# stevesuyao/KinectDepthMapEnhancement

Measured on AMD Instinct MI355X. Metric: Mpixels/sec joint-bilateral filtered (640x480 & 1080p); % HBM roofline, higher is better.
Workload: dtype f32; 1 GPU; JointBilateralFilter::Process (K0 pre-smooth 5/30/30 + K1) on 64 x 640x480 synthetic RGB-D frames (64 per GPU), window 11 (radius 5), sigma_s 3 px, sigma_r 7.65/255, sigma_d 20 mm; frames_per_gpu=64, width=640, height=480, window=11, kernel_variant=auto (w11-pk2-16x16-false-v4)

## Files before the change

### kinectdepthmapenhancement_amd/csrc/jbf_kernels.hip

```cpp
#include "kde_internal.h"
#include "kde_device_math.h"
#include "kde_device_packed.h"

namespace kde {
namespace {

constexpr int kTileX = 32;
constexpr int kTileY = 8;
constexpr int kThreads = kTileX * kTileY;

__device__ __forceinline__ int color_dist2(uint32_t a, uint32_t b)
{
    int d0 = (int)(a & 0xffu) - (int)(b & 0xffu);
    int d1 = (int)((a >> 8) & 0xffu) - (int)((b >> 8) & 0xffu);
    int d2 = (int)((a >> 16) & 0xffu) - (int)((b >> 16) & 0xffu);
    return d0 * d0 + d1 * d1 + d2 * d2;
}

__device__ __forceinline__ int reflect101(int p, int len)
{
    if (len == 1) return 0;
    while (p < 0 || p >= len) {
        if (p < 0) p = -p;
        else p = 2 * len - 2 - p;
    }
    return p;
}

struct JbfDev {
    const float* depth;
    const uint8_t* guide;
    float* out;
    const float* s_eff;
    int width, height, window;
    float color_den, depth_den;
    int color_on, depth_on;
    int cd_skip;
    float d2_skip;
    KDE_STAGE(float* stage_avg;)
};

__global__ __launch_bounds__(kThreads) void jbf_generic_kernel(JbfDev a)
{
    extern __shared__ __attribute__((aligned(16))) unsigned char smem[];
    const int R = a.window / 2;
    const int LW = kTileX + 2 * R, LH = kTileY + 2 * R;
    float* sd = reinterpret_cast<float*>(smem);
    uint32_t* sc = reinterpret_cast<uint32_t*>(sd + LW * LH);
    float* ss = reinterpret_cast<float*>(sc + LW * LH);

    const size_t frame = (size_t)blockIdx.z * a.width * a.height;
    const float* __restrict__ depth = a.depth + frame;
    const uint8_t* __restrict__ guide = a.guide + frame * 3;
    const int x0 = blockIdx.x * kTileX, y0 = blockIdx.y * kTileY;
    const int tid = threadIdx.x;

    for (int i = tid; i < LW * LH; i += kThreads) {
        const int ly = i / LW, lx = i - ly * LW;
        const int gx = x0 + lx - R, gy = y0 + ly - R;
        float d = 0.0f;
        uint32_t c = 0;
        if (gx >= 0 && gx < a.width && gy >= 0 && gy < a.height) {
            const size_t q = (size_t)gy * a.width + gx;
            d = depth[q];
            if (!(d > 50.0f)) d = 0.0f;
            c = load_bgrx(guide, q);
        }
        sd[i] = d;
        sc[i] = c;
    }
    for (int i = tid; i < a.window * a.window; i += kThreads) ss[i] = a.s_eff[i];
    __syncthreads();

    const int tx = tid & (kTileX - 1), ty = tid / kTileX;
    const int x = x0 + tx, y = y0 + ty;
    if (x >= a.width || y >= a.height) return;

    const uint32_t cc = sc[(ty + R) * LW + tx + R];
    float w_average = 0.0f, weight = 0.0f;
    for (int i = 0; i < a.window; i++) {
        for (int j = 0; j < a.window; j++) {
            const int li = (ty + i) * LW + tx + j;
            const float dq = sd[li];
            if (dq > 50.0f) {
                const int cd = color_dist2(cc, sc[li]);
                float filter = ss[i * a.window + j];
                if (a.color_on && cd < a.cd_skip) filter *= exp_denormal(-(float)cd / a.color_den);
                w_average += dq * filter;
                weight += filter;
            }
        }
    }
    float result = 0.0f;
    if (weight > 0.0f) {
        w_average /= weight;
        float numerator = 0.0f, denominator = 0.0f;
        for (int i = 0; i < a.window; i++) {
            for (int j = 0; j < a.window; j++) {
                const int li = (ty + i) * LW + tx + j;
                const float dq = sd[li];
                if (dq > 50.0f) {
                    const int cd = color_dist2(cc, sc[li]);
                    float filter = ss[i * a.window + j];
                    if (a.color_on && cd < a.cd_skip) filter *= exp_denormal(-(float)cd / a.color_den);
                    const float dd = dq - w_average;
                    const float d2 = dd * dd;
                    if (a.depth_on && !(d2 >= a.d2_skip)) filter *= exp_denormal(-d2 / a.depth_den);
                    numerator += dq * filter;
                    denominator += filter;
                }
            }
        }
        result = (denominator == 0.0f) ? 0.0f : numerator / denominator;
    }
    a.out[frame + (size_t)y * a.width + x] = result;
    KDE_STAGE(if (a.stage_avg) a.stage_avg[frame + (size_t)y * a.width + x] = weight > 0.0f ? w_average : __builtin_nanf("");)
}

struct PreDev {
    const uint8_t* src;
    uint8_t* dst;
    const float* lut;
    int width, height, n;
    int tiles_x, tiles_y;
    int band_walk;
    FastDiv24 div_tpf, div_tx;
};

constexpr int kPreBX = 16, kPreBY = 16;

__device__ __forceinline__ uint32_t cvt_pk_u8(float v, uint32_t byte, uint32_t old)
{
    uint32_t r;
    asm("v_cvt_pk_u8_f32 %0, %1, %2, %3" : "=v"(r) : "v"(v), "v"(byte), "v"(old));
    return r;
}
constexpr int kPreTH = kPreBY;

constexpr int kPreRpWaves = 7;
template <int R, int PX>
__global__ __launch_bounds__(kPreBX* kPreBY, (R <= 2 ? kPreRpWaves : 0)) void presmooth_kernel(PreDev a)
{
    constexpr int kPrePX = PX, kPreTW = kPreBX * PX;
    constexpr int NT = kPreBX * kPreBY;
    constexpr int LW = kPreTW + 2 * R, LH = kPreTH + 2 * R;
    constexpr int LUT_N = (R * R + 1) * 766;
    constexpr int SEG = kPrePX + 2 * R;
    __shared__ float lut[LUT_N];
    constexpr int LP = (LW + 3) / 4 * 4;
    __shared__ __attribute__((aligned(16))) uint32_t sc[LH * LP + 4];

    const int tid = threadIdx.x;
    for (int i = tid; i < LUT_N; i += NT) lut[i] = a.lut[i];
    const float w_centre = __uint_as_float(__builtin_amdgcn_readfirstlane(__float_as_uint(a.lut[0])));

    const int tiles_per_frame = a.tiles_x * a.tiles_y;
    const int total = tiles_per_frame * a.n;
    const int tx = tid % kPreBX, ty = tid / kPreBX;

    constexpr int RPP = NT / LW;
    constexpr int NSLOT = (LH + RPP - 1) / RPP;
    const int sy0 = tid / LW, sx = tid - sy0 * LW;
    const bool stager = sy0 < RPP;
    const uint32_t lds0 = (uint32_t)(sy0 * LP + sx);
    const uint32_t rel0 = ((uint32_t)sy0 * (uint32_t)a.width + (uint32_t)sx) * 3u;
    const uint32_t out_rel = ((uint32_t)ty * (uint32_t)a.width + (uint32_t)(tx * kPrePX)) * 3u;
    const size_t last_pix = (size_t)a.n * a.width * a.height - 1;
    auto tile_of = [&](int L) { return a.band_walk ? (int)xcd_band_id((unsigned)L, (unsigned)total) : L; };
    constexpr int kRun = 4;
    const unsigned w_xcd = blockIdx.x % 8u, w_slot = blockIdx.x / 8u;
    const unsigned w_per = (unsigned)total / 8u, w_rem = (unsigned)total % 8u;
    const unsigned w_start = w_xcd * w_per + (w_xcd < w_rem ? w_xcd : w_rem), w_len = w_per + (w_xcd < w_rem ? 1u : 0u);
    const unsigned w_wgs = (gridDim.x + 7u - w_xcd) / 8u;
    const unsigned w_full = a.band_walk == 2 ? w_len / ((unsigned)kRun * w_wgs) : 0u;
    auto tile_index = [&](int it) -> int {
        if (a.band_walk != 2) {
            const long long L = (long long)blockIdx.x + (long long)it * gridDim.x;
            return L < total ? tile_of((int)L) : -1;
        }
        unsigned pos;
        if ((unsigned)it < w_full * kRun) pos = (unsigned)kRun * (w_slot + ((unsigned)it / kRun) * w_wgs) + (unsigned)it % kRun;
        else pos = w_full * kRun * w_wgs + w_slot + ((unsigned)it - w_full * kRun) * w_wgs;
        return pos < w_len ? (int)(w_start + pos) : -1;
    };
    struct TileAt { int frame_i, tyi, txi; };
    auto tile_at = [&](int tile_id) {
        const uint32_t t = (uint32_t)tile_id;
        const uint32_t f = fastdiv24(t, a.div_tpf);
        const uint32_t tile = t - f * (uint32_t)tiles_per_frame;
        const uint32_t ty_ = fastdiv24(tile, a.div_tx);
        return TileAt{(int)f, (int)ty_, (int)(tile - ty_ * (uint32_t)a.tiles_x)};
    };
    auto fetch = [&](const TileAt& at, uint32_t* pre) {
        const int frame_i = at.frame_i, tyi = at.tyi, txi = at.txi;
        const size_t frame = (size_t)frame_i * a.width * a.height;
        const bool ends_batch = frame_i == a.n - 1 && txi * kPreTW + kPreTW + R == a.width && tyi * kPreTH + kPreTH + R == a.height;
        const bool inner = txi * kPreTW - R >= 0 && txi * kPreTW + kPreTW + R <= a.width && tyi * kPreTH - R >= 0 &&
                           tyi * kPreTH + kPreTH + R <= a.height && !ends_batch;
        if (inner) {
            const uint8_t* base = a.src + (frame + (size_t)(tyi * kPreTH - R) * a.width + (size_t)(txi * kPreTW - R)) * 3;
#pragma unroll
            for (int k = 0; k < NSLOT; k++) {
                if (stager && sy0 + k * RPP < LH)
                    __builtin_memcpy(&pre[k], base + (size_t)(k * RPP) * a.width * 3 + rel0, 4);
            }
            return;
        }
#pragma unroll
        for (int k = 0; k < NSLOT; k++) {
            if (stager && sy0 + k * RPP < LH) {
                const int gx = reflect101(txi * kPreTW + sx - R, a.width);
                const int gy = reflect101(tyi * kPreTH + sy0 + k * RPP - R, a.height);
                const size_t pix = frame + (size_t)gy * a.width + gx;
                if (pix < last_pix) __builtin_memcpy(&pre[k], a.src + pix * 3, 4);
                else pre[k] = load_bgrx(a.src, pix);
            }
        }
    };

    uint32_t pre[NSLOT];
    TileAt cur{0, 0, 0};
    int cur_id = tile_index(0);
    if (cur_id >= 0) {
        cur = tile_at(cur_id);
        fetch(cur, pre);
    }
    for (int it = 0; cur_id >= 0; it++) {
        const int frame_i = cur.frame_i;
        const int x0 = cur.txi * kPreTW, y0 = cur.tyi * kPreTH;
        const size_t frame = (size_t)frame_i * a.width * a.height;

        __syncthreads();
#pragma unroll
        for (int k = 0; k < NSLOT; k++)
            if (stager && sy0 + k * RPP < LH) sc[lds0 + k * RPP * LP] = pre[k] & 0x00ffffffu;
        __syncthreads();
        cur_id = tile_index(it + 1);
        if (cur_id >= 0) {
            cur = tile_at(cur_id);
            fetch(cur, pre);
        }

        const bool full = x0 + kPreTW <= a.width && y0 + kPreTH <= a.height;
        const int xb = x0 + tx * kPrePX, y = y0 + ty;
        if (!full && (xb >= a.width || y >= a.height)) continue;

        uint32_t cc[kPrePX];
        f2 sbg[kPrePX];
        float sr[kPrePX], sden[kPrePX];
#pragma unroll
        for (int k = 0; k < kPrePX; k++) {
            cc[k] = sc[(ty + R) * LP + tx * kPrePX + R + k];
            sbg[k] = f2{0.0f, 0.0f};
            sr[k] = sden[k] = 0.0f;
        }
#pragma unroll
        for (int dy = -R; dy <= R; dy++) {
            uint32_t v[(SEG + 3) / 4 * 4];
            f2 fbg[SEG];
            float fr[SEG];
            if (PX == 4) {
#pragma unroll
                for (int q4 = 0; q4 < (SEG + 3) / 4; q4++) {
                    const uint4 w = *reinterpret_cast<const uint4*>(&sc[(ty + R + dy) * LP + tx * kPrePX + 4 * q4]);
                    v[4 * q4] = w.x; v[4 * q4 + 1] = w.y; v[4 * q4 + 2] = w.z; v[4 * q4 + 3] = w.w;
                }
            } else {
#pragma unroll
                for (int q2 = 0; q2 < (SEG + 1) / 2; q2++) {
                    const uint2 w = *reinterpret_cast<const uint2*>(&sc[(ty + R + dy) * LP + tx * kPrePX + 2 * q2]);
                    v[2 * q2] = w.x; v[2 * q2 + 1] = w.y;
                }
            }
#pragma unroll
            for (int q = 0; q < SEG; q++) {
                fbg[q] = f2{(float)(v[q] & 0xffu), (float)((v[q] >> 8) & 0xffu)};
                fr[q] = (float)((v[q] >> 16) & 0xffu);
            }
#pragma unroll
            for (int dx = -R; dx <= R; dx++) {
                const int space2 = dx * dx + dy * dy;
                if (space2 > R * R) continue;
#pragma unroll
                for (int k = 0; k < kPrePX; k++) {
                    const int q = k + R + dx;
                    float w;
                    if (space2 == 0) {
                        w = w_centre;
                    } else {
                        const uint32_t n1 = __builtin_amdgcn_sad_u8(v[q], cc[k], 0u);
                        w = lut[space2 * 766 + n1];
                    }
                    sbg[k] = __builtin_elementwise_fma(f2{w, w}, fbg[q], sbg[k]);
                    sr[k] = __builtin_fmaf(w, fr[q], sr[k]);
                    sden[k] += w;
                }
            }
        }
        uint32_t px[kPrePX];
#pragma unroll
        for (int k = 0; k < kPrePX; k++) {
            const float den = sden[k];
            const float r = __builtin_amdgcn_rcpf(den);
            const f2 qbg = sbg[k] * f2{r, r};
            float q[3] = {qbg.x, qbg.y, sr[k] * r};
            const f2 ebg = f2{__builtin_amdgcn_fractf(q[0]), __builtin_amdgcn_fractf(q[1])} - f2{0.5f, 0.5f};
            const float er = __builtin_amdgcn_fractf(q[2]) - 0.5f;
            const float emin = __builtin_fminf(__builtin_fminf(__builtin_fabsf(ebg.x), __builtin_fabsf(ebg.y)), __builtin_fabsf(er));
            const bool ambiguous = !(emin > 1.0e-4f) || !__builtin_amdgcn_class(den, 0x100);
            if (ambiguous) {
                q[0] = sbg[k].x / den;
                q[1] = sbg[k].y / den;
                q[2] = sr[k] / den;
            }
            px[k] = cvt_pk_u8(q[2], 2u, cvt_pk_u8(q[1], 1u, cvt_pk_u8(q[0], 0u, 0u)));
        }
        uint8_t* o = a.dst + (frame + (size_t)y0 * a.width + x0) * 3 + out_rel;
        if (PX == 4 && (a.width & 3) == 0 && xb + 3 < a.width && (reinterpret_cast<uintptr_t>(a.dst) & 3u) == 0) {
            uint32_t* ow = reinterpret_cast<uint32_t*>(o);
            ow[0] = px[0] | (px[1] << 24);
            ow[1] = (px[1] >> 8) | (px[2] << 16);
            ow[2] = (px[2] >> 16) | (px[3 % PX] << 8);
        } else if (PX == 2 && (full || xb + 1 < a.width)) {
            const uint16_t h0 = (uint16_t)(px[0] & 0xffffu), h1 = (uint16_t)((px[0] >> 16) | ((px[1] & 0xffu) << 8)),
                           h2 = (uint16_t)(px[1] >> 8);
            __builtin_memcpy(o, &h0, 2);
            __builtin_memcpy(o + 2, &h1, 2);
            __builtin_memcpy(o + 4, &h2, 2);
        } else {
#pragma unroll
            for (int k = 0; k < kPrePX; k++)
                if (xb + k < a.width) {
                    o[3 * k] = (uint8_t)(px[k] & 0xff);
                    o[3 * k + 1] = (uint8_t)((px[k] >> 8) & 0xff);
                    o[3 * k + 2] = (uint8_t)((px[k] >> 16) & 0xff);
                }
        }
    }
}

__global__ __launch_bounds__(kPreBX* kPreBY) void presmooth_generic_kernel(PreDev a, int R)
{
    const int x = blockIdx.x * kPreBX + threadIdx.x % kPreBX, y = blockIdx.y * kPreBY + threadIdx.x / kPreBX;
    if (x >= a.width || y >= a.height) return;
    const size_t frame = (size_t)blockIdx.z * a.width * a.height;
    const uint32_t cc = load_bgrx(a.src, frame + (size_t)y * a.width + x);
    float s0 = 0.0f, s1 = 0.0f, s2 = 0.0f, sum2 = 0.0f;
    for (int dy = -R; dy <= R; dy++) {
        const int gy = reflect101(y + dy, a.height);
        for (int dx = -R; dx <= R; dx++) {
            const int space2 = dx * dx + dy * dy;
            if (space2 > R * R) continue;
            const uint32_t v = load_bgrx(a.src, frame + (size_t)gy * a.width + reflect101(x + dx, a.width));
            const uint32_t n1 = __builtin_amdgcn_sad_u8(v, cc, 0u);
            const float w = a.lut[(size_t)space2 * 766 + n1];
            s0 = __builtin_fmaf(w, (float)(v & 0xffu), s0);
            s1 = __builtin_fmaf(w, (float)((v >> 8) & 0xffu), s1);
            s2 = __builtin_fmaf(w, (float)((v >> 16) & 0xffu), s2);
            sum2 += w;
        }
    }
    auto sat = [](float q) -> uint8_t {
        if (!(q > 0.0f)) return 0;
        if (q >= 255.0f) return 255;
        return (uint8_t)rintf(q);
    };
    uint8_t* o = a.dst + (frame + (size_t)y * a.width + x) * 3;
    o[0] = sat(s0 / sum2);
    o[1] = sat(s1 / sum2);
    o[2] = sat(s2 / sum2);
}

struct MrfDev {
    const float* depth;
    const uint8_t* bgr;
    float* out;
    int width, height, window;
    float color_sigma, smooth_sigma;
};

__global__ __launch_bounds__(kThreads) void mrf_kernel(MrfDev a)
{
    extern __shared__ __attribute__((aligned(16))) unsigned char smem[];
    const int R = a.window / 2;
    const int LW = kTileX + 2 * R, LH = kTileY + 2 * R;
    float* sd = reinterpret_cast<float*>(smem);
    uint32_t* sc = reinterpret_cast<uint32_t*>(sd + LW * LH);

    const size_t frame = (size_t)blockIdx.z * a.width * a.height;
    const float* __restrict__ depth = a.depth + frame;
    const uint8_t* __restrict__ bgr = a.bgr + frame * 3;
    const int x0 = blockIdx.x * kTileX, y0 = blockIdx.y * kTileY;
    const int tid = threadIdx.x;

    for (int i = tid; i < LW * LH; i += kThreads) {
        const int ly = i / LW, lx = i - ly * LW;
        const int gx = x0 + lx - R, gy = y0 + ly - R;
        float d = 0.0f;
        uint32_t c = 0;
        if (gx >= 0 && gx < a.width && gy >= 0 && gy < a.height) {
            const size_t q = (size_t)gy * a.width + gx;
            d = depth[q];
            if (!(d > 50.0f)) d = 0.0f;
            c = load_bgrx(bgr, q);
        }
        sd[i] = d;
        sc[i] = c;
    }
    __syncthreads();

    const int tx = tid & (kTileX - 1), ty = tid / kTileX;
    const int x = x0 + tx, y = y0 + ty;
    if (x >= a.width || y >= a.height) return;

    const uint32_t cc = sc[(ty + R) * LW + tx + R];
    float numerator = depth[(size_t)y * a.width + x], denominator = 1.0f;
    for (int i = 0; i < a.window; i++) {
        for (int j = 0; j < a.window; j++) {
            const int li = (ty + i) * LW + tx + j;
            const float dq = sd[li];
            if (dq > 50.0f) {
                const int cd = color_dist2(cc, sc[li]);
                float color_filter = 0.0f;
                if (a.color_sigma != 0.0f) color_filter = exp_denormal(-a.color_sigma * (float)cd);
                float filter = a.smooth_sigma;
                filter *= color_filter;
                numerator += dq * filter;
                denominator += filter;
            }
        }
    }
    a.out[frame + (size_t)y * a.width + x] = (denominator == 0.0f) ? 0.0f : numerator / denominator;
}

}

int jbf_variant_count() { return 1 + jbf_fast_variant_count(); }
const char* jbf_variant_name(int v) { return v == 0 ? "generic-32x8-1px" : jbf_fast_variant_name(v - 1); }

int jbf_active_variant(const JbfLaunch& a)
{
    if (a.variant > 0) return a.variant;
    if (a.variant < 0 && jbf_fast_supported(a)) return 1 + jbf_fast_default_variant(a);
    return 0;
}

int launch_jbf(const JbfLaunch& a, hipStream_t s)
{
    if (a.variant > 0) {
        if (!jbf_fast_supported(a)) return fail(KDE_ERR_INVALID, "jbf: tuned variants need non-zero sigmas and a built window");
        return launch_jbf_fast(a, a.variant - 1, a.table_host, s);
    }
    if (a.variant < 0 && jbf_fast_supported(a))
        return launch_jbf_fast(a, jbf_fast_default_variant(a), a.table_host, s);
    JbfDev d;
    d.depth = a.depth;
    d.guide = a.guide;
    d.out = a.out;
    d.s_eff = a.s_eff;
    d.width = a.width;
    d.height = a.height;
    d.window = a.window;
    d.color_den = a.color_den;
    d.depth_den = a.depth_den;
    d.color_on = a.color_sigma != 0.0f;
    d.depth_on = a.depth_sigma != 0.0f;
    d.cd_skip = a.cd_skip;
    d.d2_skip = a.d2_skip;
    KDE_STAGE(d.stage_avg = g_stage.jbf_avg;)
    const int R = a.window / 2;
    const size_t lds = (size_t)(kTileX + 2 * R) * (kTileY + 2 * R) * 8 + (size_t)a.window * a.window * 4;
    dim3 grid(ceil_div(a.width, kTileX), ceil_div(a.height, kTileY), a.n);
    hipLaunchKernelGGL(jbf_generic_kernel, grid, dim3(kThreads), lds, s, d);
    KDE_HIP_TRY(hipGetLastError());
    return KDE_OK;
}

constexpr int kPrePxPerThread = 2;

long long presmooth_resident_blocks(int radius)
{
    auto resident = [](auto kernel) -> long long {
        int dev = 0, cus = 0, per_cu = 0;
        if (hipGetDevice(&dev) != hipSuccess ||
            hipDeviceGetAttribute(&cus, hipDeviceAttributeMultiprocessorCount, dev) != hipSuccess ||
            hipOccupancyMaxActiveBlocksPerMultiprocessor(&per_cu, kernel, kPreBX * kPreBY, 0) != hipSuccess ||
            cus <= 0 || per_cu <= 0) {
            (void)hipGetLastError();
            return 256;
        }
        return (long long)cus * per_cu;
    };
    switch (radius) {
        case 1: return resident(presmooth_kernel<1, kPrePxPerThread>);
        case 2: return resident(presmooth_kernel<2, kPrePxPerThread>);
        case 3: return resident(presmooth_kernel<3, kPrePxPerThread>);
        case 4: return resident(presmooth_kernel<4, kPrePxPerThread>);
        default: return 0;
    }
}

static int k0_band_walk(int width, int height, int n)
{
    return (long long)width * height * n * 3 <= (32ll << 20) ? 1 : 2;
}

int launch_presmooth(const PresmoothLaunch& a, hipStream_t s)
{
    PreDev d;
    d.src = a.src;
    d.dst = a.dst;
    d.lut = a.lut;
    d.width = a.width;
    d.height = a.height;
    d.n = a.n;
    constexpr int kPX = kPrePxPerThread;
    d.band_walk = k0_band_walk(a.width, a.height, a.n);
    d.tiles_x = ceil_div(a.width, kPreBX * kPX);
    d.tiles_y = ceil_div(a.height, kPreTH);
    if (a.radius < 1) return fail(KDE_ERR_INVALID, "presmooth: radius %d", a.radius);
    if (a.radius > 4) {
        if (a.n > 65535) return fail(KDE_ERR_INVALID, "presmooth: batch too large for one launch");
        hipLaunchKernelGGL(presmooth_generic_kernel, dim3(ceil_div(a.width, kPreBX), ceil_div(a.height, kPreBY), a.n),
                           dim3(kPreBX * kPreBY), 0, s, d, a.radius);
        KDE_HIP_TRY(hipGetLastError());
        return KDE_OK;
    }
    const long long total = (long long)d.tiles_x * d.tiles_y * a.n;
    if (total > 0x7fffffffLL) return fail(KDE_ERR_INVALID, "presmooth: batch too large for one launch");
    d.div_tpf = make_fastdiv24((uint32_t)(d.tiles_x * d.tiles_y), (uint64_t)total);
    d.div_tx = make_fastdiv24((uint32_t)d.tiles_x, (uint64_t)d.tiles_x * d.tiles_y);
    const long long cap = a.grid_cap > 0 ? a.grid_cap : 256;
    const unsigned grid = (unsigned)(total < cap ? total : cap);
    if (d.band_walk == 2 && grid < 8) d.band_walk = 1;
    switch (a.radius) {
        case 1: hipLaunchKernelGGL((presmooth_kernel<1, kPX>), dim3(grid), dim3(kPreBX * kPreBY), 0, s, d); break;
        case 2: hipLaunchKernelGGL((presmooth_kernel<2, kPX>), dim3(grid), dim3(kPreBX * kPreBY), 0, s, d); break;
        case 3: hipLaunchKernelGGL((presmooth_kernel<3, kPX>), dim3(grid), dim3(kPreBX * kPreBY), 0, s, d); break;
        default: hipLaunchKernelGGL((presmooth_kernel<4, kPX>), dim3(grid), dim3(kPreBX * kPreBY), 0, s, d); break;
    }
    KDE_HIP_TRY(hipGetLastError());
    return KDE_OK;
}

struct MrfFastDev {
    const float* depth;
    const uint8_t* bgr;
    float* out;
    int width, height;
    float kc;
    float lsm;
    float unscale;
};

constexpr int kMrfBX = 32, kMrfBY = 8, kMrfPX = 2;

template <int WIN>
__global__ __launch_bounds__(kMrfBX* kMrfBY) void mrf_fast_kernel(MrfFastDev a)
{
    constexpr int R = WIN / 2, NT = kMrfBX * kMrfBY, TW = kMrfBX * kMrfPX, TH = kMrfBY;
    constexpr int LW = TW + 2 * R, LH = TH + 2 * R;
    constexpr uint32_t kMagicM = 0x4B000000u, kOffM = 1u << 18, kInvalidM = 0xFF000000u;
    constexpr float kBiasM = 8388608.0f + 262144.0f;
    __shared__ __attribute__((aligned(8))) float s_d[LH * LW];
    __shared__ __attribute__((aligned(8))) uint32_t s_c[LH * LW];
    __shared__ __attribute__((aligned(8))) uint32_t s_n[LH * LW];

    const size_t frame = (size_t)blockIdx.z * a.width * a.height;
    const float* __restrict__ depth = a.depth + frame;
    const uint8_t* __restrict__ bgr = a.bgr + frame * 3;
    const int x0 = blockIdx.x * TW, y0 = blockIdx.y * TH;
    const int tid = threadIdx.x;
    for (int i = tid; i < LW * LH; i += NT) {
        const int ly = i / LW, lx = i - ly * LW;
        const int gx = x0 + lx - R, gy = y0 + ly - R;
        float d = 0.0f;
        uint32_t c = 0;
        if (gx >= 0 && gx < a.width && gy >= 0 && gy < a.height) {
            const size_t q = (size_t)gy * a.width + gx;
            d = depth[q];
            c = load_bgrx(bgr, q);
        }
        const bool valid = d > 50.0f;
        s_d[i] = valid ? d : 0.0f;
        s_c[i] = c;
        s_n[i] = valid ? (kMagicM + kOffM) - __builtin_amdgcn_udot4(c, c, 0u, false) : kInvalidM;
    }
    __syncthreads();

    const int tx = tid % kMrfBX, ty = tid / kMrfBX;
    const int xb = x0 + tx * kMrfPX, y = y0 + ty;
    if (xb >= a.width || y >= a.height) return;
    static_assert(kMrfPX == 2 && LW % 2 == 0, "pair geometry");
    constexpr int SEGP = 1 + R;
    uint32_t cc[2];
    f2 negC, num = {0.0f, 0.0f}, den = {0.0f, 0.0f};
#pragma unroll
    for (int k = 0; k < 2; k++) {
        cc[k] = s_c[(ty + R) * LW + tx * 2 + R + k];
        negC[k] = -(kBiasM + (float)__builtin_amdgcn_udot4(cc[k], cc[k], 0u, false));
    }
    const f2 kc2 = {a.kc, a.kc}, lsm2 = {a.lsm, a.lsm};
#pragma unroll
    for (int i = 0; i < WIN; i++) {
        f2 dp[SEGP];
        uint2 cp[SEGP], np[SEGP];
#pragma unroll
        for (int m = 0; m < SEGP; m++) {
            const int li = (ty + i) * LW + tx * 2 + 2 * m;
            dp[m] = *reinterpret_cast<const f2*>(&s_d[li]);
            cp[m] = *reinterpret_cast<const uint2*>(&s_c[li]);
            np[m] = *reinterpret_cast<const uint2*>(&s_n[li]);
        }
#pragma unroll
        for (int u = 0; u < WIN; u++) {
            uint32_t c0, c1, n0, n1;
            pair_unit_pick(cp, WIN, u, 0, c0, c1);
            pair_unit_pick(np, WIN, u, 0, n0, n1);
            const f2 dq = pair_unit_pick(dp, WIN, u);
            const uint32_t u0 = (__builtin_amdgcn_udot4(c0, cc[0], 0u, false) << 1) + n0;
            const uint32_t u1 = (__builtin_amdgcn_udot4(c1, cc[1], 0u, false) << 1) + n1;
            const f2 ncd = f2{__uint_as_float(u0), __uint_as_float(u1)} + negC;
            const f2 arg = __builtin_elementwise_fma(ncd, kc2, lsm2);
            const f2 f = {__builtin_amdgcn_exp2f(arg.x), __builtin_amdgcn_exp2f(arg.y)};
            num = __builtin_elementwise_fma(dq, f, num);
            den = den + f;
        }
    }
    float* __restrict__ o = a.out + frame + (size_t)y * a.width + xb;
#pragma unroll
    for (int k = 0; k < kMrfPX; k++)
        if (xb + k < a.width) {
            const float n = __builtin_fmaf(num[k], a.unscale, depth[(size_t)y * a.width + xb + k]);
            const float d = __builtin_fmaf(den[k], a.unscale, 1.0f);
            o[k] = (d == 0.0f) ? 0.0f : n / d;
        }
}

int launch_mrf(const MrfLaunch& a, hipStream_t s)
{
    if (a.window == 5 && a.color_sigma > 0.0f && a.smooth_sigma >= 0.0f && a.color_sigma < 1.0e30f && a.smooth_sigma < 1.0e30f) {
        MrfFastDev f;
        f.depth = a.depth; f.bgr = a.bgr; f.out = a.out; f.width = a.width; f.height = a.height;
        f.kc = (float)((double)a.color_sigma * 1.4426950408889634);
        const double lsm = a.smooth_sigma == 0.0f ? -INFINITY : std::log2((double)a.smooth_sigma);
        const int off = lsm + 32.0 < 120.0 ? 32 : 0;
        f.lsm = (float)(lsm + off);
        f.unscale = (float)std::ldexp(1.0, -off);
        dim3 fgrid(ceil_div(a.width, kMrfBX * kMrfPX), ceil_div(a.height, kMrfBY), a.n);
        hipLaunchKernelGGL(mrf_fast_kernel<5>, fgrid, dim3(kMrfBX * kMrfBY), 0, s, f);
        KDE_HIP_TRY(hipGetLastError());
        return KDE_OK;
    }
    MrfDev d{a.depth, a.bgr, a.out, a.width, a.height, a.window, a.color_sigma, a.smooth_sigma};
    const int R = a.window / 2;
    const size_t lds = (size_t)(kTileX + 2 * R) * (kTileY + 2 * R) * 8;
    dim3 grid(ceil_div(a.width, kTileX), ceil_div(a.height, kTileY), a.n);
    hipLaunchKernelGGL(mrf_kernel, grid, dim3(kThreads), lds, s, d);
    KDE_HIP_TRY(hipGetLastError());
    return KDE_OK;
}

}
```

Baseline: 18150 Mpixels/s.

## Pre-convert presmooth LDS tile to float4, compact LUT, faster border fetch

The presmooth kernel now stores each staged pixel in LDS as a float4 holding the three channels already converted to float plus the packed bits, so the inner loop skips per-row unpacking and int-to-float conversion. The spatial LUT is compacted to only the squared distances that actually occur, shrinking its LDS footprint. Border tiles take a cheaper reflect path using 32-bit offsets, and the exact-division fallback for ambiguous rounding is grouped behind a single branch. The cost is a 4x larger LDS tile, which raises LDS traffic and may lower occupancy.

```diff
diff --git a/kinectdepthmapenhancement_amd/csrc/jbf_kernels.hip b/kinectdepthmapenhancement_amd/csrc/jbf_kernels.hip
--- a/kinectdepthmapenhancement_amd/csrc/jbf_kernels.hip
+++ b/kinectdepthmapenhancement_amd/csrc/jbf_kernels.hip
@@ -25,6 +25,13 @@
         else p = 2 * len - 2 - p;
     }
     return p;
+}
+
+__device__ __forceinline__ int reflect_near(int p, int len)
+{
+    p = p < 0 ? -p : p;
+    p = p >= len ? 2 * len - 2 - p : p;
+    return p < 0 ? 0 : p;
 }
 
 struct JbfDev {
@@ -136,6 +143,24 @@
     return r;
 }
 constexpr int kPreTH = kPreBY;
+typedef float f4 __attribute__((ext_vector_type(4)));
+
+struct PreRowMap {
+    int row[17];
+    int n;
+};
+constexpr PreRowMap make_pre_row_map(int R)
+{
+    PreRowMap m{};
+    for (int s2 = 0; s2 < 17; s2++) m.row[s2] = -1;
+    for (int s2 = 1; s2 <= R * R; s2++) {
+        bool occurs = false;
+        for (int dy = 0; dy <= R; dy++)
+            for (int dx = 0; dx <= R; dx++) occurs = occurs || dx * dx + dy * dy == s2;
+        if (occurs) m.row[s2] = m.n++;
+    }
+    return m;
+}
 
 constexpr int kPreRpWaves = 7;
 template <int R, int PX>
@@ -144,14 +169,17 @@
     constexpr int kPrePX = PX, kPreTW = kPreBX * PX;
     constexpr int NT = kPreBX * kPreBY;
     constexpr int LW = kPreTW + 2 * R, LH = kPreTH + 2 * R;
-    constexpr int LUT_N = (R * R + 1) * 766;
     constexpr int SEG = kPrePX + 2 * R;
-    __shared__ float lut[LUT_N];
-    constexpr int LP = (LW + 3) / 4 * 4;
-    __shared__ __attribute__((aligned(16))) uint32_t sc[LH * LP + 4];
+    constexpr PreRowMap kRows = make_pre_row_map(R);
+    __shared__ float lut[kRows.n * 766];
+    constexpr int LP = LW | 1;
+    __shared__ __attribute__((aligned(16))) f4 sc[LH * LP];
 
     const int tid = threadIdx.x;
-    for (int i = tid; i < LUT_N; i += NT) lut[i] = a.lut[i];
+#pragma unroll
+    for (int s2 = 1; s2 <= R * R; s2++)
+        if (kRows.row[s2] >= 0)
+            for (int i = tid; i < 766; i += NT) lut[kRows.row[s2] * 766 + i] = a.lut[s2 * 766 + i];
     const float w_centre = __uint_as_float(__builtin_amdgcn_readfirstlane(__float_as_uint(a.lut[0])));
 
     const int tiles_per_frame = a.tiles_x * a.tiles_y;
@@ -191,6 +219,7 @@
         const uint32_t ty_ = fastdiv24(tile, a.div_tx);
         return TileAt{(int)f, (int)ty_, (int)(tile - ty_ * (uint32_t)a.tiles_x)};
     };
+    const bool border_fast = a.width > R && a.height > R && (unsigned long long)a.width * (unsigned long long)a.height * 3ull < (1ull << 32);
     auto fetch = [&](const TileAt& at, uint32_t* pre) {
         const int frame_i = at.frame_i, tyi = at.tyi, txi = at.txi;
         const size_t frame = (size_t)frame_i * a.width * a.height;
@@ -206,6 +235,22 @@
             }
             return;
         }
+        if (border_fast) {
+            const uint8_t* fbase = a.src + frame * 3;
+            const bool has_last = frame_i == a.n - 1 && txi * kPreTW + kPreTW + R >= a.width && tyi * kPreTH + kPreTH + R >= a.height;
+            const uint32_t last_off = ((uint32_t)a.width * (uint32_t)a.height - 1u) * 3u;
+            const int gx = reflect_near(txi * kPreTW + sx - R, a.width);
+#pragma unroll
+            for (int k = 0; k < NSLOT; k++) {
+                if (stager && sy0 + k * RPP < LH) {
+                    const int gy = reflect_near(tyi * kPreTH + sy0 + k * RPP - R, a.height);
+                    const uint32_t off = ((uint32_t)gy * (uint32_t)a.width + (uint32_t)gx) * 3u;
+                    if (has_last && off == last_off) pre[k] = load_bgrx(fbase, (size_t)gy * a.width + gx);
+                    else __builtin_memcpy(&pre[k], fbase + off, 4);
+                }
+            }
+            return;
+        }
 #pragma unroll
         for (int k = 0; k < NSLOT; k++) {
             if (stager && sy0 + k * RPP < LH) {
@@ -233,7 +278,10 @@
         __syncthreads();
 #pragma unroll
         for (int k = 0; k < NSLOT; k++)
-            if (stager && sy0 + k * RPP < LH) sc[lds0 + k * RPP * LP] = pre[k] & 0x00ffffffu;
+            if (stager && sy0 + k * RPP < LH) {
+                const uint32_t v = pre[k] & 0x00ffffffu;
+                sc[lds0 + k * RPP * LP] = f4{(float)(v & 0xffu), (float)((v >> 8) & 0xffu), (float)((v >> 16) & 0xffu), __uint_as_float(v)};
+            }
         __syncthreads();
         cur_id = tile_index(it + 1);
         if (cur_id >= 0) {
@@ -250,32 +298,21 @@
         float sr[kPrePX], sden[kPrePX];
 #pragma unroll
         for (int k = 0; k < kPrePX; k++) {
-            cc[k] = sc[(ty + R) * LP + tx * kPrePX + R + k];
+            cc[k] = __float_as_uint(sc[(ty + R) * LP + tx * kPrePX + R + k].w);
             sbg[k] = f2{0.0f, 0.0f};
             sr[k] = sden[k] = 0.0f;
         }
 #pragma unroll
         for (int dy = -R; dy <= R; dy++) {
-            uint32_t v[(SEG + 3) / 4 * 4];
+            uint32_t v[SEG];
             f2 fbg[SEG];
             float fr[SEG];
-            if (PX == 4) {
-#pragma unroll
-                for (int q4 = 0; q4 < (SEG + 3) / 4; q4++) {
-                    const uint4 w = *reinterpret_cast<const uint4*>(&sc[(ty + R + dy) * LP + tx * kPrePX + 4 * q4]);
-                    v[4 * q4] = w.x; v[4 * q4 + 1] = w.y; v[4 * q4 + 2] = w.z; v[4 * q4 + 3] = w.w;
-                }
-            } else {
-#pragma unroll
-                for (int q2 = 0; q2 < (SEG + 1) / 2; q2++) {
-                    const uint2 w = *reinterpret_cast<const uint2*>(&sc[(ty + R + dy) * LP + tx * kPrePX + 2 * q2]);
-                    v[2 * q2] = w.x; v[2 * q2 + 1] = w.y;
-                }
-            }
 #pragma unroll
             for (int q = 0; q < SEG; q++) {
-                fbg[q] = f2{(float)(v[q] & 0xffu), (float)((v[q] >> 8) & 0xffu)};
-                fr[q] = (float)((v[q] >> 16) & 0xffu);
+                const f4 w = sc[(ty + R + dy) * LP + tx * kPrePX + q];
+                fbg[q] = f2{w.x, w.y};
+                fr[q] = w.z;
+                v[q] = __float_as_uint(w.w);
             }
 #pragma unroll
             for (int dx = -R; dx <= R; dx++) {
@@ -289,7 +326,7 @@
                         w = w_centre;
                     } else {
                         const uint32_t n1 = __builtin_amdgcn_sad_u8(v[q], cc[k], 0u);
-                        w = lut[space2 * 766 + n1];
+                        w = lut[kRows.row[space2] * 766 + n1];
                     }
                     sbg[k] = __builtin_elementwise_fma(f2{w, w}, fbg[q], sbg[k]);
                     sr[k] = __builtin_fmaf(w, fr[q], sr[k]);
@@ -298,23 +335,33 @@
             }
         }
         uint32_t px[kPrePX];
+        float q[kPrePX][3];
+        bool ambiguous[kPrePX], any_ambiguous = false;
 #pragma unroll
         for (int k = 0; k < kPrePX; k++) {
             const float den = sden[k];
             const float r = __builtin_amdgcn_rcpf(den);
             const f2 qbg = sbg[k] * f2{r, r};
-            float q[3] = {qbg.x, qbg.y, sr[k] * r};
-            const f2 ebg = f2{__builtin_amdgcn_fractf(q[0]), __builtin_amdgcn_fractf(q[1])} - f2{0.5f, 0.5f};
-            const float er = __builtin_amdgcn_fractf(q[2]) - 0.5f;
+            q[k][0] = qbg.x;
+            q[k][1] = qbg.y;
+            q[k][2] = sr[k] * r;
+            const f2 ebg = f2{__builtin_amdgcn_fractf(q[k][0]), __builtin_amdgcn_fractf(q[k][1])} - f2{0.5f, 0.5f};
+            const float er = __builtin_amdgcn_fractf(q[k][2]) - 0.5f;
             const float emin = __builtin_fminf(__builtin_fminf(__builtin_fabsf(ebg.x), __builtin_fabsf(ebg.y)), __builtin_fabsf(er));
-            const bool ambiguous = !(emin > 1.0e-4f) || !__builtin_amdgcn_class(den, 0x100);
-            if (ambiguous) {
-                q[0] = sbg[k].x / den;
-                q[1] = sbg[k].y / den;
-                q[2] = sr[k] / den;
-            }
-            px[k] = cvt_pk_u8(q[2], 2u, cvt_pk_u8(q[1], 1u, cvt_pk_u8(q[0], 0u, 0u)));
-        }
+            ambiguous[k] = !(emin > 1.0e-4f) || !__builtin_amdgcn_classf(den, 0x100);
+            any_ambiguous = any_ambiguous || ambiguous[k];
+        }
+        if (any_ambiguous) {
+#pragma unroll
+            for (int k = 0; k < kPrePX; k++)
+                if (ambiguous[k]) {
+                    q[k][0] = sbg[k].x / sden[k];
+                    q[k][1] = sbg[k].y / sden[k];
+                    q[k][2] = sr[k] / sden[k];
+                }
+        }
+#pragma unroll
+        for (int k = 0; k < kPrePX; k++) px[k] = cvt_pk_u8(q[k][2], 2u, cvt_pk_u8(q[k][1], 1u, cvt_pk_u8(q[k][0], 0u, 0u)));
         uint8_t* o = a.dst + (frame + (size_t)y0 * a.width + x0) * 3 + out_rel;
         if (PX == 4 && (a.width & 3) == 0 && xb + 3 < a.width && (reinterpret_cast<uintptr_t>(a.dst) & 3u) == 0) {
             uint32_t* ow = reinterpret_cast<uint32_t*>(o);
```

Result: no change. 18300 Mpixels/s (median of 6 runs) (+0.8%).
